# Alexander-H-Liu/End-to-end-ASR-Pytorch

Measured on AMD Instinct MI355X. Metric: audio frames/sec training (LAS+CTC, LibriSpeech 80-mel), higher is better.
Workload: dtype f32; 1 GPU; cfg3: {"B": 32, "T": 1600, "D": 80, "V": 5000, "L": 64}; global_batch=32, parallelism=dp1

## Files before the change

end-to-end-asr-pytorch_amd/csrc/core.cpp:

```cpp
#include "common.h"
#include "knobs.h"
#include <cstdlib>
#include <mutex>
#include <vector>

namespace {
struct DevInfo {
    int cu_count = 0;
    int lds_per_cu = 0;
    bool ok = false;
};
DevInfo g_dev[64];

struct ProfRec {
    hipEvent_t a, b;
    int id;
};
bool g_prof_on = false;
std::vector<ProfRec> g_pending;
double g_total_ms[PROF_NUM];
int64_t g_launches[PROF_NUM];
std::mutex g_mu;
hipEvent_t g_cur[PROF_NUM];
}

namespace {
AsrkKnobs g_knobs;
std::once_flag g_knobs_once;
int env_int(const char *name) {
    const char *e = getenv(name);
    return e ? atoi(e) : AsrkKnobs::UNSET;
}
int env_present(const char *name) { return getenv(name) ? 1 : AsrkKnobs::UNSET; }
void read_knobs() {
    AsrkKnobs &k = g_knobs;
    k.gemm_noskinny = env_present("ASRK_GEMM_NOSKINNY");
    k.skinny_sk = env_int("ASRK_SKINNY_SK");
    k.gemm_dbg = env_int("ASRK_GEMM_DBG");
    k.gemm_nofast = env_present("ASRK_GEMM_NOFAST");
    k.split_w256 = env_int("ASRK_SPLIT_W256");
    k.split_tail = env_int("ASRK_SPLIT_TAIL");
    k.fwd_mt = env_int("ASRK_FWD_MT");
    k.fwd_nt = env_int("ASRK_FWD_NT");
    k.rec_bf_mt4 = env_int("ASRK_REC_BF_MT4");
    k.bwd_ub = env_int("ASRK_BWD_UB");
    k.bwd_nt = env_int("ASRK_BWD_NT");
    k.fwd_poll = env_int("ASRK_FWD_POLL");
    k.fwd_presleep = env_int("ASRK_FWD_PRESLEEP");
    k.bwd_poll = env_int("ASRK_BWD_POLL");
    k.bwd_presleep = env_int("ASRK_BWD_PRESLEEP");
    k.dbg_noload = env_present("ASRK_DBG_NOLOAD");
    k.deterministic = env_int("ASRK_DETERMINISTIC");
}
}

const AsrkKnobs &asrk_knobs_() {
    std::call_once(g_knobs_once, read_knobs);
    return g_knobs;
}

extern "C" int asrk_version(void) { return 200; }

extern "C" const char *asrk_strerror(int rc) {
    switch (rc) {
        case ASRK_OK: return "ok";
        case ASRK_EINVAL: return "asrk: invalid argument";
        case ASRK_ESHAPE: return "asrk: shape not supported by the persistent gfx950 kernels";
        case ASRK_EWORKSPACE: return "asrk: workspace too small";
        case ASRK_EDEVICE: return "asrk: device lacks the CUs/LDS the persistent kernel needs";
        case ASRK_ETIMEOUT: return "asrk: in-kernel grid synchronisation timed out";
        default: break;
    }
    if (rc > 0) return hipGetErrorString((hipError_t)rc);
    return "asrk: unknown error";
}

extern "C" int asrk_init(int device) {
    if (device < 0 || device >= 64) return ASRK_EINVAL;
    (void)asrk_knobs_();
    if (!g_dev[device].ok) {
        hipDeviceProp_t prop;
        hipError_t e = hipGetDeviceProperties(&prop, device);
        if (e != hipSuccess) return (int)e > 0 ? -(1000 + (int)e) : ASRK_EDEVICE;
        g_dev[device].cu_count = prop.multiProcessorCount;
        g_dev[device].lds_per_cu = (int)prop.maxSharedMemoryPerMultiProcessor;
        g_dev[device].ok = true;
    }
    return g_dev[device].cu_count;
}

extern "C" int asrk_cu_count_(void) {
    int dev = 0;
    if (hipGetDevice(&dev) != hipSuccess) return 0;
    if (dev < 0 || dev >= 64) return 0;
    if (!g_dev[dev].ok) {
        if (asrk_init(dev) <= 0) return 0;
    }
    return g_dev[dev].cu_count;
}

static double g_work[PROF_NUM] = {0};

static unsigned g_prof_mask = 0xffffffffu;
extern "C" void asrk_profile_enable(int on) { g_prof_on = on != 0; }
extern "C" void asrk_profile_families(unsigned mask) { g_prof_mask = mask; }
static inline bool prof_live(int id) { return g_prof_on && id >= 0 && id < PROF_NUM && ((g_prof_mask >> id) & 1u); }

extern "C" void asrk_profile_reset(void) {
    std::lock_guard<std::mutex> lk(g_mu);
    for (auto &r : g_pending) {
        hipEventDestroy(r.a);
        hipEventDestroy(r.b);
    }
    g_pending.clear();
    for (int i = 0; i < PROF_NUM; ++i) {
        g_total_ms[i] = 0.0;
        g_launches[i] = 0;
        g_work[i] = 0.0;
    }
}

extern "C" void asrk_prof_work_(int id, double flops) {
    if (prof_live(id)) g_work[id] += flops;
}
extern "C" int asrk_profile_get_work(int id, double *flops) {
    if (id < 0 || id >= PROF_NUM || !flops) return ASRK_EINVAL;
    *flops = g_work[id];
    return ASRK_OK;
}

extern "C" void asrk_prof_begin_(int id, hipStream_t s) {
    if (!prof_live(id)) return;
    hipEvent_t a;
    if (hipEventCreate(&a) != hipSuccess) return;
    hipEventRecord(a, s);
    g_cur[id] = a;
}

extern "C" void asrk_prof_end_(int id, hipStream_t s) {
    if (!prof_live(id)) return;
    hipEvent_t b;
    if (hipEventCreate(&b) != hipSuccess) return;
    hipEventRecord(b, s);
    std::lock_guard<std::mutex> lk(g_mu);
    g_pending.push_back({g_cur[id], b, id});
}

extern "C" void asrk_prof_launches_(int id, int64_t n) {
    if (!prof_live(id)) return;
    std::lock_guard<std::mutex> lk(g_mu);
    g_launches[id] += n;
}

extern "C" int asrk_profile_get(int id, double *total_ms, int64_t *launches) {
    if (id < 0 || id >= PROF_NUM) return ASRK_EINVAL;
    std::lock_guard<std::mutex> lk(g_mu);
    for (auto &r : g_pending) {
        hipEventSynchronize(r.b);
        float ms = 0.f;
        if (hipEventElapsedTime(&ms, r.a, r.b) == hipSuccess) {
            g_total_ms[r.id] += ms;
            g_launches[r.id] += 1;
        }
        hipEventDestroy(r.a);
        hipEventDestroy(r.b);
    }
    g_pending.clear();
    if (total_ms) *total_ms = g_total_ms[id];
    if (launches) *launches = g_launches[id];
    return ASRK_OK;
}
```

end-to-end-asr-pytorch_amd/csrc/gemm_split.hip:

```cpp
#include "common.h"
#include "knobs.h"
#include <algorithm>
#include <climits>

extern "C" int asrk_cu_count_(void);

namespace {

typedef __bf16 bf16x8 __attribute__((ext_vector_type(8)));

constexpr int PIECE = 1024;

struct SplitGemmArgs {
    const unsigned char *Ap, *Bp;
    float *C;
    const float *bias, *bias2;
    int M, N, ldc;
    int KC;
    size_t rb_stride_a, rb_stride_b;
    int nk;
    int tiles_m, tiles_n;
    float alpha, beta;
    int slices, ldw;
    float *ws;
};

__device__ __forceinline__ void split8(const float (&v)[8], u32x4 (&w)[3]) {
    unsigned h[3][8];
#pragma unroll
    for (int e = 0; e < 8; ++e) {
        const float a = v[e];
        const __bf16 b0 = (__bf16)a;
        const float r1 = a - (float)b0;
        const __bf16 b1 = (__bf16)r1;
        const float r2 = r1 - (float)b1;
        const __bf16 b2 = (__bf16)r2;
        h[0][e] = __builtin_bit_cast(unsigned short, b0);
        h[1][e] = __builtin_bit_cast(unsigned short, b1);
        h[2][e] = __builtin_bit_cast(unsigned short, b2);
    }
#pragma unroll
    for (int p = 0; p < 3; ++p)
#pragma unroll
        for (int q = 0; q < 4; ++q) w[p][q] = h[p][2 * q] | (h[p][2 * q + 1] << 16);
}

template <bool VEC>
__global__ __launch_bounds__(256) void split_panel_kernel(const float *__restrict__ src, int ld, int R, int K,
                                                          unsigned char *__restrict__ dst, int KC, int RB,
                                                          size_t rb_stride) {
    constexpr int CHUNK = 3 * PIECE;
    const int lane = threadIdx.x & 63;
    const int KG = KC >> 2;
    const int64_t item = (int64_t)blockIdx.x * 4 + (threadIdx.x >> 6);
    if (item >= (int64_t)RB * KG) return;
    const int rb = (int)(item / KG), c0 = (int)(item - (int64_t)rb * KG) * 4;
    unsigned char *drb = dst + (size_t)rb * rb_stride;
    const int c = c0 + (lane & 3), k0 = c * 8;
#pragma unroll
    for (int it = 0; it < 4; ++it) {
        const int rl = it * 16 + (lane >> 2), row = rb * 64 + rl;
        float v[8];
        const float *s = src + (size_t)row * ld + k0;
        if (VEC && row < R && k0 + 8 <= K) {
            const f32x4 lo = *reinterpret_cast<const f32x4 *>(s), hi = *reinterpret_cast<const f32x4 *>(s + 4);
            v[0] = lo[0]; v[1] = lo[1]; v[2] = lo[2]; v[3] = lo[3];
            v[4] = hi[0]; v[5] = hi[1]; v[6] = hi[2]; v[7] = hi[3];
        } else {
#pragma unroll
            for (int e = 0; e < 8; ++e) v[e] = (row < R && k0 + e < K) ? s[e] : 0.f;
        }
        u32x4 w[3];
        split8(v, w);
        unsigned char *d = drb + (size_t)c * CHUNK + rl * 16;
#pragma unroll
        for (int p = 0; p < 3; ++p) *reinterpret_cast<u32x4 *>(d + p * PIECE) = w[p];
    }
}

template <int NCG>
__global__ __launch_bounds__(256) void split_panel_t_kernel(const float *__restrict__ src, int ld, int R, int K,
                                                            unsigned char *__restrict__ dst, int KC, int RB,
                                                            size_t rb_stride) {
    constexpr int CHUNK = 3 * PIECE;
    const int lane = threadIdx.x & 63, wave = __builtin_amdgcn_readfirstlane(threadIdx.x >> 6);
    const int64_t item = (int64_t)blockIdx.x * 4 + wave;
    const int KGn = KC / NCG;
    if (item >= (int64_t)RB * KGn) return;
    const int g = (int)(item / RB), rb = (int)(item - (int64_t)g * RB);
    const int c0 = g * NCG, k0 = c0 * 8, row = rb * 64 + lane;
    float v[NCG][8];
    const float *s = src + (size_t)k0 * ld + row;
    if (k0 + 8 * NCG <= K && rb * 64 + 64 <= R) {
#pragma unroll
        for (int cc = 0; cc < NCG; ++cc)
#pragma unroll
            for (int e = 0; e < 8; ++e) v[cc][e] = s[(size_t)(cc * 8 + e) * ld];
    } else {
#pragma unroll
        for (int cc = 0; cc < NCG; ++cc)
#pragma unroll
            for (int e = 0; e < 8; ++e)
                v[cc][e] = (row < R && k0 + cc * 8 + e < K) ? s[(size_t)(cc * 8 + e) * ld] : 0.f;
    }
    unsigned char *d = dst + (size_t)rb * rb_stride + (size_t)c0 * CHUNK + lane * 16;
#pragma unroll
    for (int cc = 0; cc < NCG; ++cc) {
        u32x4 w[3];
        split8(v[cc], w);
#pragma unroll
        for (int p = 0; p < 3; ++p) *reinterpret_cast<u32x4 *>(d + (size_t)cc * CHUNK + p * PIECE) = w[p];
    }
}

template <int N>
__device__ __forceinline__ void glds16_run(const unsigned char *g, unsigned voff, unsigned char *l) {
    static_assert(N >= 1 && N <= 4, "immediate offset range");
    const auto *gp = (const __attribute__((address_space(1))) unsigned char *)g + voff;
    auto *lp = (__attribute__((address_space(3))) void *)l;
    __builtin_amdgcn_global_load_lds(gp, lp, 16, 0, 0);
    if constexpr (N > 1) __builtin_amdgcn_global_load_lds(gp, lp, 16, PIECE, 0);
    if constexpr (N > 2) __builtin_amdgcn_global_load_lds(gp, lp, 16, 2 * PIECE, 0);
    if constexpr (N > 3) __builtin_amdgcn_global_load_lds(gp, lp, 16, 3 * PIECE, 0);
}

template <int N>
__device__ __forceinline__ void wait_vm() {
    static_assert(N >= 0 && N < 64, "vmcnt is a 6-bit field");
    __builtin_amdgcn_s_waitcnt((N & 15) | 0x70 | 0xF00 | (((N >> 4) & 3) << 14));
}
__device__ __forceinline__ void wait_lgkm0() { __builtin_amdgcn_s_waitcnt(0xC07F); }

template <int NC, int NST, bool SPEC, int WM, bool SK = false>
__global__ __launch_bounds__(SPEC ? (WM == 2 ? 512 : 704) : 256) void gemm_bf16x6_kernel(SplitGemmArgs p) {
    extern __shared__ __attribute__((aligned(1024))) unsigned char lds[];
    static_assert(WM == 2 || (WM == 4 && SPEC), "256-row tiles only with DMA waves");
    static_assert(!SK || NST >= 2, "the split-K epilogue transposes through a stage the last k-tile does not use");
    constexpr int NPL = 3, CHUNK = NPL * PIECE;
    constexpr int NCW = 2 * WM;
    constexpr int NRG = WM + 2;
    constexpr int RPD = WM == 2 ? 1 : 2;
    constexpr int REGION = NC * CHUNK;
    constexpr int STAGE = NRG * REGION;
    constexpr int LPT = NC * NPL * RPD;
    const int tid = threadIdx.x, lane = tid & 63;
    const int wave = __builtin_amdgcn_readfirstlane(tid >> 6);
    const int ntiles = p.tiles_m * p.tiles_n;
    const int slice = SK ? blockIdx.x / ntiles : 0, bid = SK ? blockIdx.x - slice * ntiles : blockIdx.x;
    const int kt0 = SK ? (int)((long)slice * p.nk / p.slices) : 0;
    const int nk = SK ? (int)((long)(slice + 1) * p.nk / p.slices) - kt0 : p.nk;
    const int q8 = ntiles >> 3, r8 = ntiles & 7, xcd = bid & 7, loc = bid >> 3;
    const int tile = (xcd < r8 ? xcd * (q8 + 1) : r8 * (q8 + 1) + (xcd - r8) * q8) + loc;
    constexpr int BAND = 8;
    const int band = tile / (BAND * p.tiles_m);
    const int band_w = min(BAND, p.tiles_n - band * BAND);
    const int in_band = tile - band * BAND * p.tiles_m;
    const int tm = in_band / band_w, tn = band * BAND + in_band % band_w;

    const bool loader = !SPEC || wave >= NCW, worker = !SPEC || wave < NCW;
    const int wr = worker ? wave >> 1 : 0, wc = wave & 1;
    const int ltm = tm, ltn = tn;
    const int r0 = (SPEC ? wave - NCW : wave) * RPD;
    const unsigned char *gsrc[RPD];
#pragma unroll
    for (int q = 0; q < RPD; ++q) {
        const int r = r0 + q;
        gsrc[q] = (r < WM ? p.Ap + (size_t)(ltm * WM + r) * p.rb_stride_a
                          : p.Bp + (size_t)(ltn * 2 + r - WM) * p.rb_stride_b);
        if (SK) gsrc[q] += (size_t)kt0 * REGION;
    }
    const unsigned voff = lane * 16;
    unsigned char *ldst = lds + r0 * REGION;
    static_assert((NC * NPL) % 4 == 0, "a region is issued as runs of four pieces");
    auto issue = [&](int kt, int stage) {
        unsigned char *l = ldst + stage * STAGE;
#pragma unroll
        for (int q = 0; q < RPD; ++q) {
            const unsigned char *g = gsrc[q] + (size_t)kt * REGION;
#pragma unroll
            for (int j = 0; j < NC * NPL; j += 4) glds16_run<4>(g + j * PIECE, voff, l + q * REGION + j * PIECE);
        }
    };

    f32x16 acc[2][2];
#pragma unroll
    for (int i = 0; i < 2; ++i)
#pragma unroll
        for (int j = 0; j < 2; ++j)
#pragma unroll
            for (int r = 0; r < 16; ++r) acc[i][j][r] = 0.f;

    const int frag_off = ((lane >> 5) * NPL) * PIECE + (lane & 31) * 16;
    const unsigned char *abase = lds + wr * REGION + frag_off;
    const unsigned char *bbase = lds + (WM + wc) * REGION + frag_off;
    constexpr int S = NC / 2;

    bf16x8 fa[2][2][NPL], fb[2][2][NPL];
    auto load_frags = [&](int buf, int stage, int ks) {
        const unsigned char *a_st = abase + stage * STAGE + ks * 2 * NPL * PIECE;
        const unsigned char *b_st = bbase + stage * STAGE + ks * 2 * NPL * PIECE;
#pragma unroll
        for (int i = 0; i < 2; ++i)
#pragma unroll
            for (int pl = 0; pl < NPL; ++pl) {
                fa[buf][i][pl] = *reinterpret_cast<const bf16x8 *>(a_st + pl * PIECE + i * 512);
                fb[buf][i][pl] = *reinterpret_cast<const bf16x8 *>(b_st + pl * PIECE + i * 512);
            }
        __builtin_amdgcn_sched_barrier(0);
    };
    auto step = [&](int buf, bool load, int lstage, int lks) {
        constexpr int NT = 6;
        constexpr int PA[6] = {2, 1, 0, 1, 0, 0};
        constexpr int PB[6] = {0, 1, 2, 0, 1, 0};
        constexpr int RPL[6] = {2, 0, 1, 1, 0, 2};
        const unsigned char *a_st = abase + lstage * STAGE + lks * 2 * NPL * PIECE;
        const unsigned char *b_st = bbase + lstage * STAGE + lks * 2 * NPL * PIECE;
        const int nb = buf ^ 1;
#pragma unroll
        for (int m = 0; m < 4 * NT; ++m) {
            const int t = m >> 2, i = (m >> 1) & 1, j = m & 1;
            acc[i][j] = __builtin_amdgcn_mfma_f32_32x32x16_bf16(fa[buf][i][PA[t]], fb[buf][j][PB[t]], acc[i][j], 0, 0, 0);
            __builtin_amdgcn_sched_barrier(0);
            if (load && m < 4 * NPL) {
                const int g = m >> 1, h = m & 1, pl = RPL[g];
                if ((g & 1) == 0) fa[nb][h][pl] = *reinterpret_cast<const bf16x8 *>(a_st + pl * PIECE + h * 512);
                else fb[nb][h][pl] = *reinterpret_cast<const bf16x8 *>(b_st + pl * PIECE + h * 512);
                __builtin_amdgcn_sched_barrier(0);
            }
        }
    };

    if (loader) {
#pragma unroll
        for (int s = 0; s < NST; ++s)
            if (s < nk) issue(s, s);
        const int later = min(NST - 1, nk - 1);
        if (NST > 3 && later >= 3) wait_vm<(NST > 3 ? 3 * LPT : 0)>();
        else if (NST > 2 && later == 2) wait_vm<(NST > 2 ? 2 * LPT : 0)>();
        else if (later == 1) wait_vm<LPT>();
        else wait_vm<0>();
    }
    __builtin_amdgcn_s_barrier();
    if (SPEC && !worker) {
        int stage = 0;
        for (int kt = 0; kt + 1 < nk; ++kt) {
            const int later = min(NST - 2, nk - 2 - kt);
            if (NST > 3 && later >= 2) wait_vm<(NST > 3 ? 2 * LPT : 0)>();
            else if (NST > 2 && later == 1) wait_vm<(NST > 2 ? LPT : 0)>();
            else wait_vm<0>();
            __builtin_amdgcn_s_barrier();
            if (kt + NST < nk) issue(kt + NST, stage);
            if (++stage == NST) stage = 0;
        }
        return;
    }
    load_frags(0, 0, 0);

    int stage = 0;
    static_assert(S >= 2 && S % 2 == 0, "fragment double buffer assumes an even number of steps per tile");
    for (int kt = 0; kt + 1 < nk; ++kt) {
#pragma unroll
        for (int ks = 0; ks < S - 1; ++ks) {
            wait_lgkm0();
            step(ks & 1, true, stage, ks + 1);
        }
        int nstage = stage + 1;
        if (nstage == NST) nstage = 0;
        const int later = min(NST - 2, nk - 2 - kt);
        wait_lgkm0();
        if (!SPEC) {
            if (NST > 3 && later >= 2) wait_vm<(NST > 3 ? 2 * LPT : 0)>();
            else if (NST > 2 && later == 1) wait_vm<(NST > 2 ? LPT : 0)>();
            else wait_vm<0>();
        }
        __builtin_amdgcn_s_barrier();
        if (!SPEC && kt + NST < nk) issue(kt + NST, stage);
        step((S - 1) & 1, true, nstage, 0);
        stage = nstage;
    }
    {
#pragma unroll
        for (int ks = 0; ks < S - 1; ++ks) {
            wait_lgkm0();
            step(ks & 1, true, stage, ks + 1);
        }
        wait_lgkm0();
        step((S - 1) & 1, false, 0, 0);
    }

    if constexpr (SK) {
        constexpr int PITCH = 36;
        static_assert(NCW * 32 * PITCH * 4 <= STAGE, "transposition images fit one stage");
        int fstage = stage + 1;
        if (fstage == NST) fstage = 0;
        float *img = reinterpret_cast<float *>(lds + fstage * STAGE) + wave * 32 * PITCH;
        float *wsl = p.ws + (size_t)slice * p.M * p.ldw;
        const int wrow0 = tm * 64 * WM + wr * 64, wcol0 = tn * 128 + wc * 64;
#pragma unroll
        for (int i = 0; i < 2; ++i)
#pragma unroll
            for (int j = 0; j < 2; ++j) {
#pragma unroll
                for (int r = 0; r < 16; ++r)
                    img[((r & 3) + 8 * (r >> 2) + 4 * (lane >> 5)) * PITCH + (lane & 31)] = acc[i][j][r];
                __builtin_amdgcn_fence(__ATOMIC_RELEASE, "wavefront");
                __builtin_amdgcn_wave_barrier();
                __builtin_amdgcn_fence(__ATOMIC_ACQUIRE, "wavefront");
#pragma unroll
                for (int q = 0; q < 4; ++q) {
                    const int idx = q * 64 + lane, rl = idx >> 3, c4 = (idx & 7) * 4;
                    const f32x4 v = *reinterpret_cast<const f32x4 *>(img + rl * PITCH + c4);
                    const int row = wrow0 + i * 32 + rl, col = wcol0 + j * 32 + c4;
                    if (row < p.M && col < p.ldw) *reinterpret_cast<f32x4 *>(wsl + (size_t)row * p.ldw + col) = v;
                }
                __builtin_amdgcn_fence(__ATOMIC_RELEASE, "wavefront");
                __builtin_amdgcn_wave_barrier();
                __builtin_amdgcn_fence(__ATOMIC_ACQUIRE, "wavefront");
            }
        return;
    }
    const int row0 = tm * 64 * WM + wr * 64 + 4 * (lane >> 5), col0 = tn * 128 + wc * 64 + (lane & 31);
#pragma unroll
    for (int j = 0; j < 2; ++j) {
        const int col = col0 + j * 32;
        if (col >= p.N) continue;
        float bsum = 0.f;
        if (p.bias) bsum += p.bias[col];
        if (p.bias2) bsum += p.bias2[col];
#pragma unroll
        for (int i = 0; i < 2; ++i)
#pragma unroll
            for (int r = 0; r < 16; ++r) {
                const int row = row0 + i * 32 + (r & 3) + 8 * (r >> 2);
                if (row >= p.M) continue;
                float *c = p.C + (size_t)row * p.ldc + col;
                float v = p.alpha * acc[i][j][r] + bsum;
                if (p.beta != 0.f) v += p.beta * *c;
                *c = v;
            }
    }
}

__global__ __launch_bounds__(256) void splitk_reduce_kernel(const float *__restrict__ ws, int slices, int M, int N,
                                                            int ldw, float alpha, float beta, float *__restrict__ C,
                                                            int ldc, const float *__restrict__ bias,
                                                            const float *__restrict__ bias2) {
    const int n4 = ldw >> 2;
    const int64_t idx = (int64_t)blockIdx.x * 256 + threadIdx.x;
    if (idx >= (int64_t)M * n4) return;
    const int row = (int)(idx / n4), col = (int)(idx - (int64_t)row * n4) * 4;
    const size_t plane = (size_t)M * ldw;
    const float *w = ws + (size_t)row * ldw + col;
    f32x4 a = *reinterpret_cast<const f32x4 *>(w);
    for (int s = 1; s < slices; ++s) a += *reinterpret_cast<const f32x4 *>(w + (size_t)s * plane);
#pragma unroll
    for (int e = 0; e < 4; ++e) {
        if (col + e >= N) break;
        float bsum = 0.f;
        if (bias) bsum += bias[col + e];
        if (bias2) bsum += bias2[col + e];
        float *c = C + (size_t)row * ldc + col + e;
        float v = alpha * a[e] + bsum;
        if (beta != 0.f) v += beta * *c;
        *c = v;
    }
}

template <int NST, int NDW>
__global__ __launch_bounds__((4 + NDW) * 64) void gemm_bf16x6_w256_kernel(SplitGemmArgs p, int rb_b, int BAND) {
    extern __shared__ __attribute__((aligned(1024))) unsigned char lds[];
    constexpr int NPL = 3, NC = 2, CHUNK = NPL * PIECE;
    constexpr int REGION = NC * CHUNK;
    constexpr int NRG = 6;
    constexpr int STAGE = NRG * REGION;
    constexpr int LPT = NRG * NC * NPL / NDW;
    static_assert(LPT * NDW == NRG * NC * NPL && (NDW == 3 || NDW == 4), "36 pieces per stage over 3 or 4 DMA waves");
    const int tid = threadIdx.x, lane = tid & 63;
    const int wave = __builtin_amdgcn_readfirstlane(tid >> 6);
    const int ntiles = p.tiles_m * p.tiles_n, bid = blockIdx.x;
    const int q8 = ntiles >> 3, r8 = ntiles & 7, xcd = bid & 7, loc = bid >> 3;
    const int tile = (xcd < r8 ? xcd * (q8 + 1) : r8 * (q8 + 1) + (xcd - r8) * q8) + loc;
    const int band = tile / (BAND * p.tiles_m);
    const int band_w = min(BAND, p.tiles_n - band * BAND);
    const int in_band = tile - band * BAND * p.tiles_m;
    const int tm = in_band / band_w, tn = band * BAND + in_band % band_w;
    const int nk = p.nk;

    if (wave >= 4) {
        const int d = wave - 4, first = d * LPT;
        constexpr int NRUN = LPT / 3;
        static_assert(NRUN * 3 == LPT, "runs of three pieces");
        const unsigned char *run_g[NRUN];
#pragma unroll
        for (int k = 0; k < NRUN; ++k) {
            const int idx = first + 3 * k, r = idx / (NC * NPL), j = idx - r * (NC * NPL);
            run_g[k] = (r < 2 ? p.Ap + (size_t)(tm * 2 + r) * p.rb_stride_a
                              : p.Bp + (size_t)min(tn * 4 + r - 2, rb_b - 1) * p.rb_stride_b) + j * PIECE;
        }
        const unsigned voff = lane * 16;
        unsigned char *ldst = lds + first * PIECE;
        auto issue = [&](int kt, int stage) {
            unsigned char *l = ldst + stage * STAGE;
            const size_t gk = (size_t)kt * REGION;
#pragma unroll
            for (int k = 0; k < NRUN; ++k) glds16_run<3>(run_g[k] + gk, voff, l + 3 * k * PIECE);
        };
#pragma unroll
        for (int s = 0; s < NST; ++s)
            if (s < nk) issue(s, s);
        {
            const int later = min(NST - 2, nk - 2);
            if (later >= 2) wait_vm<2 * LPT>();
            else if (later == 1) wait_vm<LPT>();
            else wait_vm<0>();
        }
        __builtin_amdgcn_s_barrier();
        int stage = 0;
        for (int kt = 0; kt < nk; ++kt) {
            const int later = min(NST - 2, nk - 2 - kt);
            if (later >= 2) wait_vm<2 * LPT>();
            else if (later == 1) wait_vm<LPT>();
            else wait_vm<0>();
            __builtin_amdgcn_s_barrier();
            if (kt + NST < nk) issue(kt + NST, stage);
            if (++stage == NST) stage = 0;
        }
        return;
    }

    const int wr = wave >> 1, wc = wave & 1;
    f32x16 acc[2][4];
#pragma unroll
    for (int i = 0; i < 2; ++i)
#pragma unroll
        for (int j = 0; j < 4; ++j)
#pragma unroll
            for (int r = 0; r < 16; ++r) acc[i][j][r] = 0.f;
    const int frag_off = ((lane >> 5) * NPL) * PIECE + (lane & 31) * 16;
    const unsigned char *abase = lds + wr * REGION + frag_off;
    const unsigned char *bbase = lds + (2 + wc * 2) * REGION + frag_off;
    bf16x8 fa1[2], fa2[2], fb1[4], fb2[4], fa0[2][2], fb0[2][4];
    auto rd_a1 = [&](bf16x8 &dst, int stage, int pl, int i) {
        dst = *reinterpret_cast<const bf16x8 *>(abase + stage * STAGE + pl * PIECE + i * 512);
    };
    auto rd_b1 = [&](bf16x8 &dst, int stage, int pl, int j) {
        dst = *reinterpret_cast<const bf16x8 *>(bbase + stage * STAGE + (j >> 1) * REGION + pl * PIECE + (j & 1) * 512);
    };
    auto rd_a = [&](bf16x8 (&dst)[2], int stage, int pl) {
#pragma unroll
        for (int i = 0; i < 2; ++i) rd_a1(dst[i], stage, pl, i);
    };
    auto rd_b = [&](bf16x8 (&dst)[4], int stage, int pl) {
#pragma unroll
        for (int j = 0; j < 4; ++j) rd_b1(dst[j], stage, pl, j);
    };
#define ASRK_TERM8(FA, FB)                                                                                 \
    do {                                                                                                   \
        _Pragma("unroll") for (int i = 0; i < 2; ++i) _Pragma("unroll") for (int j = 0; j < 4; ++j)         \
            acc[i][j] = __builtin_amdgcn_mfma_f32_32x32x16_bf16(FA[i], FB[j], acc[i][j], 0, 0, 0);          \
        __builtin_amdgcn_sched_barrier(0);                                                                 \
    } while (0)
#define ASRK_TERM8_RD(FA, FB, RD)                                                                          \
    do {                                                                                                   \
        _Pragma("unroll") for (int m = 0; m < 8; ++m) {                                                    \
            acc[m >> 2][m & 3] =                                                                           \
                __builtin_amdgcn_mfma_f32_32x32x16_bf16(FA[m >> 2], FB[m & 3], acc[m >> 2][m & 3], 0, 0, 0); \
            __builtin_amdgcn_sched_barrier(0);                                                             \
            RD(m);                                                                                         \
            __builtin_amdgcn_sched_barrier(0);                                                             \
        }                                                                                                  \
    } while (0)
#define ASRK_STEP(P)                                                                                       \
    do {                                                                                                   \
        int nstage = stage + 1;                                                                            \
        if (nstage == NST) nstage = 0;                                                                     \
        ASRK_TERM8(fa2, fb0[P]);                                                                           \
        wait_lgkm0();                                                                                      \
        __builtin_amdgcn_s_barrier();                                           \
        auto rd2 = [&](int m) {                                                                            \
            if (m == 0) rd_a1(fa2[0], nstage, 2, 0);                                                       \
            else if (m == 2) rd_a1(fa2[1], nstage, 2, 1);                                                  \
            else if (m == 4) rd_b1(fb0[1 - (P)][0], nstage, 0, 0);                                         \
            else if (m == 6) rd_b1(fb0[1 - (P)][1], nstage, 0, 1);                                         \
        };                                                                                                 \
        ASRK_TERM8_RD(fa0[P], fb2, rd2);                                                                   \
        auto rd3 = [&](int m) {                                                                            \
            if ((m & 1) == 0) rd_b1(fb2[m >> 1], nstage, 2, m >> 1);                                       \
        };                                                                                                 \
        ASRK_TERM8_RD(fa0[P], fb1, rd3);                                                                   \
        auto rd4 = [&](int m) {                                                                            \
            if (m == 0) rd_b1(fb0[1 - (P)][2], nstage, 0, 2);                                              \
            else if (m == 2) rd_b1(fb0[1 - (P)][3], nstage, 0, 3);                                         \
            else if (m == 4) rd_a1(fa0[1 - (P)][0], nstage, 0, 0);                                         \
            else if (m == 6) rd_a1(fa0[1 - (P)][1], nstage, 0, 1);                                         \
        };                                                                                                 \
        ASRK_TERM8_RD(fa1, fb1, rd4);                                                                      \
        auto rd5 = [&](int m) {                                                                            \
            if ((m & 1) == 0) rd_b1(fb1[m >> 1], nstage, 1, m >> 1);                                       \
        };                                                                                                 \
        ASRK_TERM8_RD(fa1, fb0[P], rd5);                                                                   \
        auto rd6 = [&](int m) {                                                                            \
            if (m == 1) rd_a1(fa1[0], nstage, 1, 0);                                                       \
            else if (m == 4) rd_a1(fa1[1], nstage, 1, 1);                                                  \
        };                                                                                                 \
        ASRK_TERM8_RD(fa0[P], fb0[P], rd6);                                                                \
        stage = nstage;                                                                                    \
    } while (0)

    __builtin_amdgcn_s_barrier();
    rd_a(fa2, 0, 2); rd_b(fb0[0], 0, 0); rd_a(fa0[0], 0, 0); rd_b(fb2, 0, 2); rd_b(fb1, 0, 1); rd_a(fa1, 0, 1);
    int stage = 0;
    for (int kt = 0; kt < nk; kt += 2) {
        ASRK_STEP(0);
        ASRK_STEP(1);
    }
#undef ASRK_STEP
#undef ASRK_TERM8_RD
#undef ASRK_TERM8

    const int row0 = tm * 128 + wr * 64 + 4 * (lane >> 5), col0 = tn * 256 + wc * 128 + (lane & 31);
#pragma unroll
    for (int j = 0; j < 4; ++j) {
        const int col = col0 + j * 32;
        if (col >= p.N) continue;
        float bsum = 0.f;
        if (p.bias) bsum += p.bias[col];
        if (p.bias2) bsum += p.bias2[col];
#pragma unroll
        for (int i = 0; i < 2; ++i)
#pragma unroll
            for (int r = 0; r < 16; ++r) {
                const int row = row0 + i * 32 + (r & 3) + 8 * (r >> 2);
                if (row >= p.M) continue;
                float *c = p.C + (size_t)row * p.ldc + col;
                float v = p.alpha * acc[i][j][r] + bsum;
                if (p.beta != 0.f) v += p.beta * *c;
                *c = v;
            }
    }
}

template <int NST, int NDW>
int launch_split_gemm_w256(const SplitGemmArgs &a, int rb_b, hipStream_t s) {
    constexpr int lds = NST * 6 * 2 * 3 * PIECE;
    auto kern = gemm_bf16x6_w256_kernel<NST, NDW>;
    static AsrkLdsLatch latch;
    ASRK_HIP(asrk_max_lds_once(latch, reinterpret_cast<const void *>(kern), lds));
    const int band = 2;
    hipLaunchKernelGGL(kern, dim3(a.tiles_m * a.tiles_n), dim3((4 + NDW) * 64), lds, s, a, rb_b, band);
    ASRK_LAUNCH_CHECK();
    return ASRK_OK;
}

template <int NC, int NST, bool SPEC, int WM, bool SK = false>
int launch_split_gemm(const SplitGemmArgs &a, hipStream_t s) {
    constexpr int lds = NST * (WM + 2) * NC * 3 * PIECE;
    auto kern = gemm_bf16x6_kernel<NC, NST, SPEC, WM, SK>;
    static AsrkLdsLatch latch;
    ASRK_HIP(asrk_max_lds_once(latch, reinterpret_cast<const void *>(kern), lds));
    hipLaunchKernelGGL(kern, dim3(a.tiles_m * a.tiles_n * (SK ? a.slices : 1)), dim3(SPEC ? (WM == 2 ? 512 : 704) : 256),
                       lds, s, a);
    ASRK_LAUNCH_CHECK();
    if (SK) {
        const int64_t items = (int64_t)a.M * (a.ldw >> 2);
        hipLaunchKernelGGL(splitk_reduce_kernel, dim3((unsigned)asrk_div_up64(items, 256)), dim3(256), 0, s, a.ws,
                           a.slices, a.M, a.N, a.ldw, a.alpha, a.beta, a.C, a.ldc, a.bias, a.bias2);
        ASRK_LAUNCH_CHECK();
    }
    return ASRK_OK;
}

}

namespace {
constexpr int SPLIT_NC = 4;
constexpr int NPL = 3;

struct PanelGeom {
    int KC, rb;
    size_t rb_stride, bytes;
};
PanelGeom panel_geom(int rows, int K, bool slack = false) {
    PanelGeom g;
    g.KC = (asrk_div_up(K, 8 * SPLIT_NC) + (slack ? 1 : 0)) * SPLIT_NC;
    g.rb = asrk_div_up(rows, 128) * 2;
    g.rb_stride = (size_t)g.KC * NPL * PIECE + 4352;
    g.bytes = (size_t)g.rb * g.rb_stride;
    return g;
}

int run_split(const float *src, int ld, int rows, int K, bool trans, unsigned char *dstp, const PanelGeom &g,
              hipStream_t s) {
    const dim3 grid((unsigned)asrk_div_up64((int64_t)g.rb * (g.KC / 4), 4));
    asrk_prof_work_(PROF_SPLIT, 4.0 * (double)rows * (double)K + 6.0 * (double)g.rb * 64.0 * (double)g.KC * 8.0);
    asrk_prof_begin_(PROF_SPLIT, s);
    if (trans) {
        hipLaunchKernelGGL((split_panel_t_kernel<4>), grid, dim3(256), 0, s, src, ld, rows, K, dstp, g.KC, g.rb, g.rb_stride);
    } else {
        const bool vec = (reinterpret_cast<uintptr_t>(src) & 15) == 0 && ld % 4 == 0;
        if (vec) hipLaunchKernelGGL((split_panel_kernel<true>), grid, dim3(256), 0, s, src, ld, rows, K, dstp, g.KC, g.rb, g.rb_stride);
        else hipLaunchKernelGGL((split_panel_kernel<false>), grid, dim3(256), 0, s, src, ld, rows, K, dstp, g.KC, g.rb, g.rb_stride);
    }
    asrk_prof_end_(PROF_SPLIT, s);
    ASRK_LAUNCH_CHECK();
    return ASRK_OK;
}

int auto_slices(int M, int N, int nk) {
    if (N >= 512) return 1;
    const int ncu = asrk_cu_count_() > 0 ? asrk_cu_count_() : 256;
    const long tiles = (long)asrk_div_up(M, 128) * asrk_div_up(N, 128);
    const long want = (ncu + tiles - 1) / tiles;
    return (int)std::max(1L, std::min(want, (long)(nk / 64)));
}

int run_panel_gemm(int M, int N, int nk, float alpha, const unsigned char *Ap, size_t stride_a,
                   const unsigned char *Bp, size_t stride_b, float beta, float *C, int ldc, const float *bias,
                   const float *bias2, hipStream_t s, int slices = 1, float *ws = nullptr) {
    const AsrkKnobs &kn = asrk_knobs_();
    SplitGemmArgs a;
    a.Ap = Ap; a.Bp = Bp; a.C = C; a.bias = bias; a.bias2 = bias2;
    a.M = M; a.N = N; a.ldc = ldc; a.KC = 0; a.nk = nk; a.rb_stride_a = stride_a; a.rb_stride_b = stride_b;
    a.tiles_m = asrk_div_up(M, 128); a.tiles_n = asrk_div_up(N, 128);
    a.alpha = alpha; a.beta = beta;
    a.slices = std::min(slices, nk); a.ldw = (N + 3) & ~3; a.ws = ws;
    if (a.slices > 1) return launch_split_gemm<4, 3, true, 2, true>(a, s);
    const int w256 = kn.get(kn.split_w256, 1);
    if (w256 && N >= 512) {
        const int tm = asrk_div_up(M, 128), tn = asrk_div_up(N, 256);
        const int ncu = asrk_cu_count_() > 0 ? asrk_cu_count_() : 256;
        if (w256 == 2 || (long)tm * tn >= 2L * ncu) {
            SplitGemmArgs b = a;
            b.tiles_m = tm; b.tiles_n = tn; b.nk = 2 * nk;
            const long tiles = (long)tm * tn, rem = tiles % ncu;
            const int tm1 = (int)((tiles - rem) / tn);
            if (w256 == 1 && rem > 0 && rem * 10 < 6L * ncu && tm1 > 0 && tm1 < tm && kn.get(kn.split_tail, 1)) {
                b.tiles_m = tm1; b.M = tm1 * 128;
                int rc = launch_split_gemm_w256<4, 4>(b, 2 * asrk_div_up(N, 128), s);
                if (rc != ASRK_OK) return rc;
                SplitGemmArgs c = a;
                c.Ap = a.Ap + (size_t)tm1 * 2 * a.rb_stride_a;
                c.C = a.C + (size_t)tm1 * 128 * ldc;
                c.M = M - tm1 * 128;
                c.tiles_m = asrk_div_up(c.M, 128);
                return launch_split_gemm<4, 3, true, 2>(c, s);
            }
            return launch_split_gemm_w256<4, 4>(b, 2 * asrk_div_up(N, 128), s);
        }
    }
    return launch_split_gemm<4, 3, true, 2>(a, s);
}
}

extern "C" size_t asrk_split_panel_stride_(int rows, int K) { return panel_geom(rows, K, true).rb_stride; }

extern "C" int asrk_gemm_takes_split(int M, int N, int K, int flags) {
    const int mode = flags & 3;
    if (mode == ASRK_GEMM_SPLIT_OFF || mode == 3 || K < 8 || M < 1 || N < 1) return 0;
    if (mode == ASRK_GEMM_SPLIT_AUTO) {
        const double hm = 2.0 * (double)M * (double)N / ((double)M + (double)N);
        const bool shallow_ok = K >= 64 && (double)M * (double)N >= 134217728.0;
        if (hm < 1500.0 || (K < 256 && !shallow_ok) || M < 256 || N < 256) return 0;
    }
    return 1;
}

extern "C" size_t asrk_gemm_ws_bytes(int M, int N, int K, int flags) {
    if (!asrk_gemm_takes_split(M, N, K, flags)) return 0;
    return panel_geom(M, K).bytes + panel_geom(N, K).bytes;
}

extern "C" int asrk_gemm_split_run_(int transA, int transB, int M, int N, int K, float alpha, const float *A,
                                    int lda, const float *B, int ldb, float beta, float *C, int ldc,
                                    const float *bias, const float *bias2, void *wsp, int flags, hipStream_t s) {
    const PanelGeom ga = panel_geom(M, K), gb = panel_geom(N, K);
    unsigned char *ws = reinterpret_cast<unsigned char *>(wsp);
    unsigned char *Ap = ws, *Bp = ws + ga.bytes;
    int rc = run_split(A, lda, M, K, transA != 0, Ap, ga, s);
    if (rc != ASRK_OK) return rc;
    rc = run_split(B, ldb, N, K, transB == 0, Bp, gb, s);
    if (rc != ASRK_OK) return rc;
    return run_panel_gemm(M, N, ga.KC / SPLIT_NC, alpha, Ap, ga.rb_stride, Bp, gb.rb_stride, beta, C, ldc, bias,
                          bias2, s);
}

extern "C" size_t asrk_split_panel_bytes(int rows, int K, int flags) {
    if (rows <= 0 || K <= 0 || flags != 0) return 0;
    return panel_geom(rows, K, true).bytes;
}

extern "C" int asrk_split_panel_f32(const float *src, int ld, int rows, int K, int trans, void *panel, int flags,
                                    void *stream) {
    if (!src || !panel || rows <= 0 || K <= 0 || ld < (trans ? rows : K) || flags != 0) return ASRK_EINVAL;
    if ((reinterpret_cast<uintptr_t>(panel) & 15) != 0) return ASRK_EINVAL;
    asrk_prof_begin_(PROF_GEMM, (hipStream_t)stream);
    const int rc = run_split(src, ld, rows, K, trans != 0, reinterpret_cast<unsigned char *>(panel),
                             panel_geom(rows, K, true), (hipStream_t)stream);
    asrk_prof_end_(PROF_GEMM, (hipStream_t)stream);
    return rc;
}

namespace {
struct PanelRange {
    const unsigned char *Ap, *Bp;
    size_t stride_a, stride_b;
    int nk;
};
int panel_range(int M, int N, int K, const void *A_panel, int a_rows, int a_K, int a_row0, int a_k0,
                const void *B_panel, int b_rows, int b_K, int b_row0, int b_k0, const float *C, int ldc, int flags,
                PanelRange &r) {
    if (M <= 0 || N <= 0 || K <= 0 || !A_panel || !B_panel || !C || ldc < N || flags != 0) return ASRK_EINVAL;
    if (a_row0 < 0 || b_row0 < 0 || a_k0 < 0 || b_k0 < 0 || a_row0 % 128 || b_row0 % 128 || a_k0 % 8 || b_k0 % 8)
        return ASRK_EINVAL;
    if (a_row0 + M > a_rows || b_row0 + N > b_rows || a_k0 + K > a_K || b_k0 + K > b_K) return ASRK_EINVAL;
    if (K % 32 != 0 && a_k0 + K != a_K && b_k0 + K != b_K) return ASRK_ESHAPE;
    const PanelGeom ga = panel_geom(a_rows, a_K, true), gb = panel_geom(b_rows, b_K, true);
    r.nk = asrk_div_up(K, 32);
    if (a_k0 / 8 + r.nk * SPLIT_NC > ga.KC || b_k0 / 8 + r.nk * SPLIT_NC > gb.KC) return ASRK_ESHAPE;
    const unsigned char *A0 = reinterpret_cast<const unsigned char *>(A_panel);
    const unsigned char *B0 = reinterpret_cast<const unsigned char *>(B_panel);
    r.Ap = A0 + (size_t)(a_row0 / 64) * ga.rb_stride + (size_t)(a_k0 / 8) * NPL * PIECE;
    r.Bp = B0 + (size_t)(b_row0 / 64) * gb.rb_stride + (size_t)(b_k0 / 8) * NPL * PIECE;
    r.stride_a = ga.rb_stride; r.stride_b = gb.rb_stride;
    return ASRK_OK;
}
}

extern "C" int asrk_gemm_panels_f32(int M, int N, int K, float alpha, const void *A_panel, int a_rows, int a_K,
                                    int a_row0, int a_k0, const void *B_panel, int b_rows, int b_K, int b_row0,
                                    int b_k0, float beta, float *C, int ldc, const float *bias,
                                    const float *bias2, int flags, void *stream) {
    PanelRange r;
    const int rc0 = panel_range(M, N, K, A_panel, a_rows, a_K, a_row0, a_k0, B_panel, b_rows, b_K, b_row0, b_k0, C, ldc,
                                flags, r);
    if (rc0 != ASRK_OK) return rc0;
    hipStream_t s = (hipStream_t)stream;
    asrk_prof_work_(PROF_GEMM, 2.0 * (double)M * (double)N * (double)K);
    asrk_prof_begin_(PROF_GEMM, s);
    const int rc = run_panel_gemm(M, N, r.nk, alpha, r.Ap, r.stride_a, r.Bp, r.stride_b, beta, C, ldc, bias, bias2, s);
    asrk_prof_end_(PROF_GEMM, s);
    return rc;
}

extern "C" size_t asrk_gemm_panels_splitk_ws_bytes(int M, int N, int splitk) {
    if (M <= 0 || N <= 0 || splitk < 0) return 0;
    const int n = splitk > 0 ? splitk : auto_slices(M, N, INT_MAX);
    return (size_t)n * (size_t)M * (size_t)((N + 3) & ~3) * sizeof(float);
}

extern "C" int asrk_gemm_panels_splitk_f32(int M, int N, int K, float alpha, const void *A_panel, int a_rows, int a_K,
                                           int a_row0, int a_k0, const void *B_panel, int b_rows, int b_K,
                                           int b_row0, int b_k0, float beta, float *C, int ldc, const float *bias,
                                           const float *bias2, int splitk, void *ws, size_t ws_bytes, int flags,
                                           void *stream) {
    if (splitk < 0 || !ws || (reinterpret_cast<uintptr_t>(ws) & 15) != 0) return ASRK_EINVAL;
    PanelRange r;
    const int rc0 = panel_range(M, N, K, A_panel, a_rows, a_K, a_row0, a_k0, B_panel, b_rows, b_K, b_row0, b_k0, C, ldc,
                                flags, r);
    if (rc0 != ASRK_OK) return rc0;
    const int slices = splitk > 0 ? splitk : auto_slices(M, N, r.nk);
    if (ws_bytes < asrk_gemm_panels_splitk_ws_bytes(M, N, slices)) return ASRK_EWORKSPACE;
    hipStream_t s = (hipStream_t)stream;
    asrk_prof_work_(PROF_GEMM, 2.0 * (double)M * (double)N * (double)K);
    asrk_prof_begin_(PROF_GEMM, s);
    const int rc = run_panel_gemm(M, N, r.nk, alpha, r.Ap, r.stride_a, r.Bp, r.stride_b, beta, C, ldc, bias, bias2, s,
                                  slices, reinterpret_cast<float *>(ws));
    asrk_prof_end_(PROF_GEMM, s);
    return rc;
}
```

end-to-end-asr-pytorch_amd/csrc/knobs.h:

```cpp
#pragma once

struct AsrkKnobs {
    static constexpr int UNSET = -0x7fffffff;
    int gemm_noskinny;
    int skinny_sk;
    int gemm_dbg;
    int gemm_nofast;
    int split_w256;
    int split_tail;
    int fwd_mt, fwd_nt;
    int rec_bf_mt4;
    int bwd_ub, bwd_nt;
    int fwd_poll, fwd_presleep;
    int bwd_poll, bwd_presleep;
    int dbg_noload;
    int deterministic;

    int get(int v, int dflt) const { return v == UNSET ? dflt : v; }
    bool is_set(int v) const { return v != UNSET; }
};

const AsrkKnobs &asrk_knobs_();
```

Before: 535,800 frames/s.

## Add 16x16x32 MFMA variants of split bf16x6 GEMM kernels for deep K

Adds new 128x128 and 128x256 split-bf16 GEMM kernels built on the 16x16x32 bf16 MFMA instruction. They interleave each MFMA with LDS fragment reads under scheduling barriers and split the waves into dedicated loader and worker groups. These kernels are selected by default when the K-panel count is at least 48, and can be overridden with an env knob. The aim is higher MFMA throughput and better overlap of LDS reads with math, at the cost of more register pressure and a large new code path.

Result: faster. 548,300 frames/s, median of 6 (+2.3%).

```diff
diff --git a/end-to-end-asr-pytorch_amd/csrc/core.cpp b/end-to-end-asr-pytorch_amd/csrc/core.cpp
--- a/end-to-end-asr-pytorch_amd/csrc/core.cpp
+++ b/end-to-end-asr-pytorch_amd/csrc/core.cpp
@@ -40,6 +40,7 @@
     k.gemm_nofast = env_present("ASRK_GEMM_NOFAST");
     k.split_w256 = env_int("ASRK_SPLIT_W256");
     k.split_tail = env_int("ASRK_SPLIT_TAIL");
+    k.split_mfma = env_int("ASRK_SPLIT_MFMA");
     k.fwd_mt = env_int("ASRK_FWD_MT");
     k.fwd_nt = env_int("ASRK_FWD_NT");
     k.rec_bf_mt4 = env_int("ASRK_REC_BF_MT4");
diff --git a/end-to-end-asr-pytorch_amd/csrc/gemm_split.hip b/end-to-end-asr-pytorch_amd/csrc/gemm_split.hip
--- a/end-to-end-asr-pytorch_amd/csrc/gemm_split.hip
+++ b/end-to-end-asr-pytorch_amd/csrc/gemm_split.hip
@@ -552,6 +552,345 @@
     return ASRK_OK;
 }
 
+#define ASRK_P16(FA, FB, ACC, RD)                                                                          \
+    do {                                                                                                   \
+        _Pragma("unroll") for (int m = 0; m < 16; ++m) {                                                   \
+            ACC[m >> 2][m & 3] =                                                                           \
+                __builtin_amdgcn_mfma_f32_16x16x32_bf16(FA[m >> 2], FB[m & 3], ACC[m >> 2][m & 3], 0, 0, 0); \
+            __builtin_amdgcn_sched_barrier(0);                                                             \
+            RD(m);                                                                                         \
+            __builtin_amdgcn_sched_barrier(0);                                                             \
+        }                                                                                                  \
+    } while (0)
+
+template <int START, int STRIDE>
+__device__ __forceinline__ void rd16_at(int m, bf16x8 (&slot)[4], const unsigned char *src) {
+    static_assert(START + 3 * STRIDE < 16, "inside one product");
+    const int i = (m - START) / STRIDE;
+    if (m >= START && i < 4 && START + i * STRIDE == m) slot[i] = *reinterpret_cast<const bf16x8 *>(src + i * 256);
+}
+__device__ __forceinline__ void rd16_all(bf16x8 (&slot)[4], const unsigned char *src) {
+#pragma unroll
+    for (int i = 0; i < 4; ++i) slot[i] = *reinterpret_cast<const bf16x8 *>(src + i * 256);
+}
+
+template <int P> struct StepSet { static constexpr int value = P; };
+
+template <bool SK>
+__global__ __launch_bounds__(512) void gemm_bf16x6_m16_kernel(SplitGemmArgs p) {
+    extern __shared__ __attribute__((aligned(1024))) unsigned char lds[];
+    constexpr int NPL = 3, NC = 4, NST = 3, CHUNK = NPL * PIECE;
+    constexpr int REGION = NC * CHUNK, STAGE = 4 * REGION, LPT = NC * NPL;
+    const int tid = threadIdx.x, lane = tid & 63;
+    const int wave = __builtin_amdgcn_readfirstlane(tid >> 6);
+    const int ntiles = p.tiles_m * p.tiles_n;
+    const int slice = SK ? blockIdx.x / ntiles : 0, bid = SK ? blockIdx.x - slice * ntiles : blockIdx.x;
+    const int kt0 = SK ? (int)((long)slice * p.nk / p.slices) : 0;
+    const int nk = SK ? (int)((long)(slice + 1) * p.nk / p.slices) - kt0 : p.nk;
+    const int q8 = ntiles >> 3, r8 = ntiles & 7, xcd = bid & 7, loc = bid >> 3;
+    const int tile = (xcd < r8 ? xcd * (q8 + 1) : r8 * (q8 + 1) + (xcd - r8) * q8) + loc;
+    constexpr int BAND = 8;
+    const int band = tile / (BAND * p.tiles_m);
+    const int band_w = min(BAND, p.tiles_n - band * BAND);
+    const int in_band = tile - band * BAND * p.tiles_m;
+    const int tm = in_band / band_w, tn = band * BAND + in_band % band_w;
+
+    const bool worker = wave < 4;
+    const int wr = worker ? wave >> 1 : 0, wc = wave & 1;
+    const int r0 = worker ? 0 : wave - 4;
+    const unsigned char *gsrc = (r0 < 2 ? p.Ap + (size_t)(tm * 2 + r0) * p.rb_stride_a
+                                        : p.Bp + (size_t)(tn * 2 + r0 - 2) * p.rb_stride_b) + (size_t)kt0 * REGION;
+    const unsigned voff = lane * 16;
+    unsigned char *ldst = lds + r0 * REGION;
+    auto issue = [&](int kt, int stage) {
+        const unsigned char *g = gsrc + (size_t)kt * REGION;
+        unsigned char *l = ldst + stage * STAGE;
+#pragma unroll
+        for (int j = 0; j < LPT; j += 4) glds16_run<4>(g + j * PIECE, voff, l + j * PIECE);
+    };
+
+    f32x4 acc[4][4];
+#pragma unroll
+    for (int i = 0; i < 4; ++i)
+#pragma unroll
+        for (int j = 0; j < 4; ++j)
+#pragma unroll
+            for (int r = 0; r < 4; ++r) acc[i][j][r] = 0.f;
+    const int frag_off = ((lane >> 4) * NPL) * PIECE + (lane & 15) * 16;
+    const unsigned char *abase = lds + wr * REGION + frag_off;
+    const unsigned char *bbase = lds + (2 + wc) * REGION + frag_off;
+    bf16x8 fa0[2][4], fa1[4], fa2[4], fb0[4], fb1[4], fb2[4];
+
+    if (!worker) {
+#pragma unroll
+        for (int s = 0; s < NST; ++s)
+            if (s < nk) issue(s, s);
+        const int later = min(NST - 1, nk - 1);
+        if (later >= 2) wait_vm<2 * LPT>();
+        else if (later == 1) wait_vm<LPT>();
+        else wait_vm<0>();
+    }
+    __builtin_amdgcn_s_barrier();
+    if (worker) {
+        rd16_all(fa0[0], abase); rd16_all(fb2, bbase + 2 * PIECE);
+        rd16_all(fa1, abase + PIECE); rd16_all(fb1, bbase + PIECE); rd16_all(fa2, abase + 2 * PIECE);
+        __builtin_amdgcn_sched_barrier(0);
+    }
+
+    int stage = 0, kt = 0;
+    auto step = [&](auto set) {
+        constexpr int P = decltype(set)::value, Q = 1 - P;
+        int nstage = stage + 1;
+        if (nstage == NST) nstage = 0;
+        const unsigned char *bc = bbase + stage * STAGE;
+        const unsigned char *an = abase + nstage * STAGE, *bn = bbase + nstage * STAGE;
+        if (worker) {
+            auto rd1 = [&](int m) { rd16_at<0, 4>(m, fb0, bc); };
+            ASRK_P16(fa0[P], fb2, acc, rd1);
+            auto rd2 = [&](int) {};
+            ASRK_P16(fa1, fb1, acc, rd2);
+            wait_lgkm0();
+        } else {
+            if (nk - 2 - kt >= 1) wait_vm<LPT>();
+            else wait_vm<0>();
+        }
+        __builtin_amdgcn_s_barrier();
+        if (worker) {
+            auto rd3 = [&](int m) { rd16_at<0, 4>(m, fb2, bn + 2 * PIECE); };
+            ASRK_P16(fa0[P], fb1, acc, rd3);
+            auto rd4 = [&](int m) { rd16_at<0, 4>(m, fa0[Q], an); };
+            ASRK_P16(fa2, fb0, acc, rd4);
+            auto rd5 = [&](int m) { rd16_at<0, 4>(m, fa2, an + 2 * PIECE); rd16_at<2, 4>(m, fb1, bn + PIECE); };
+            ASRK_P16(fa1, fb0, acc, rd5);
+            auto rd6 = [&](int m) { rd16_at<0, 2>(m, fa1, an + PIECE); };
+            ASRK_P16(fa0[P], fb0, acc, rd6);
+        } else if (kt + NST < nk) {
+            issue(kt + NST, stage);
+        }
+        stage = nstage;
+        ++kt;
+    };
+    while (kt < nk) {
+        step(StepSet<0>());
+        if (kt < nk) step(StepSet<1>());
+    }
+    if (!worker) return;
+
+    if constexpr (SK) {
+        constexpr int PITCH = 68;
+        static_assert(4 * 16 * PITCH * 4 <= STAGE, "transposition images fit one stage");
+        float *img = reinterpret_cast<float *>(lds) + wave * 16 * PITCH;
+        float *wsl = p.ws + (size_t)slice * p.M * p.ldw;
+        const int wrow0 = tm * 128 + wr * 64, wcol0 = tn * 128 + wc * 64;
+        wait_lgkm0();
+#pragma unroll
+        for (int i = 0; i < 4; ++i) {
+#pragma unroll
+            for (int j = 0; j < 4; ++j)
+#pragma unroll
+                for (int r = 0; r < 4; ++r) img[(4 * (lane >> 4) + r) * PITCH + j * 16 + (lane & 15)] = acc[i][j][r];
+            __builtin_amdgcn_fence(__ATOMIC_RELEASE, "wavefront");
+            __builtin_amdgcn_wave_barrier();
+            __builtin_amdgcn_fence(__ATOMIC_ACQUIRE, "wavefront");
+#pragma unroll
+            for (int q = 0; q < 4; ++q) {
+                const int idx = q * 64 + lane, rl = idx >> 4, c4 = (idx & 15) * 4;
+                const f32x4 v = *reinterpret_cast<const f32x4 *>(img + rl * PITCH + c4);
+                const int row = wrow0 + i * 16 + rl, col = wcol0 + c4;
+                if (row < p.M && col < p.ldw) *reinterpret_cast<f32x4 *>(wsl + (size_t)row * p.ldw + col) = v;
+            }
+            __builtin_amdgcn_fence(__ATOMIC_RELEASE, "wavefront");
+            __builtin_amdgcn_wave_barrier();
+            __builtin_amdgcn_fence(__ATOMIC_ACQUIRE, "wavefront");
+        }
+        return;
+    }
+    const int row0 = tm * 128 + wr * 64 + 4 * (lane >> 4), col0 = tn * 128 + wc * 64 + (lane & 15);
+#pragma unroll
+    for (int j = 0; j < 4; ++j) {
+        const int col = col0 + j * 16;
+        if (col >= p.N) continue;
+        float bsum = 0.f;
+        if (p.bias) bsum += p.bias[col];
+        if (p.bias2) bsum += p.bias2[col];
+#pragma unroll
+        for (int i = 0; i < 4; ++i)
+#pragma unroll
+            for (int r = 0; r < 4; ++r) {
+                const int row = row0 + i * 16 + r;
+                if (row >= p.M) continue;
+                float *c = p.C + (size_t)row * p.ldc + col;
+                float v = p.alpha * acc[i][j][r] + bsum;
+                if (p.beta != 0.f) v += p.beta * *c;
+                *c = v;
+            }
+    }
+}
+
+template <int NDW>
+__global__ __launch_bounds__((4 + NDW) * 64) void gemm_bf16x6_w256_m16_kernel(SplitGemmArgs p, int rb_b, int BAND) {
+    extern __shared__ __attribute__((aligned(1024))) unsigned char lds[];
+    constexpr int NPL = 3, NC = 2, CHUNK = NPL * PIECE;
+    constexpr int REGION = NC * CHUNK, NRG = 6, STAGE = NRG * REGION, PAIR = 2 * STAGE;
+    constexpr int LPT = NRG * NC * NPL / NDW, NRUN = LPT / 3;
+    static_assert(LPT * NDW == NRG * NC * NPL && NRUN * 3 == LPT, "36 pieces per stage, runs of three");
+    const int tid = threadIdx.x, lane = tid & 63;
+    const int wave = __builtin_amdgcn_readfirstlane(tid >> 6);
+    const int ntiles = p.tiles_m * p.tiles_n, bid = blockIdx.x;
+    const int q8 = ntiles >> 3, r8 = ntiles & 7, xcd = bid & 7, loc = bid >> 3;
+    const int tile = (xcd < r8 ? xcd * (q8 + 1) : r8 * (q8 + 1) + (xcd - r8) * q8) + loc;
+    const int band = tile / (BAND * p.tiles_m);
+    const int band_w = min(BAND, p.tiles_n - band * BAND);
+    const int in_band = tile - band * BAND * p.tiles_m;
+    const int tm = in_band / band_w, tn = band * BAND + in_band % band_w;
+    const int ns = p.nk >> 1;
+
+    const bool worker = wave < 4;
+    const int first = (worker ? 0 : wave - 4) * LPT;
+    const unsigned char *run_g[NRUN];
+#pragma unroll
+    for (int k = 0; k < NRUN; ++k) {
+        const int idx = first + 3 * k, r = idx / (NC * NPL), j = idx - r * (NC * NPL);
+        run_g[k] = (r < 2 ? p.Ap + (size_t)(tm * 2 + r) * p.rb_stride_a
+                          : p.Bp + (size_t)min(tn * 4 + r - 2, rb_b - 1) * p.rb_stride_b) + j * PIECE;
+    }
+    const unsigned voff = lane * 16;
+    unsigned char *ldst = lds + first * PIECE;
+    auto issue_pair = [&](int s, int slot) {
+#pragma unroll
+        for (int h = 0; h < 2; ++h) {
+            unsigned char *l = ldst + slot * PAIR + h * STAGE;
+            const size_t gk = (size_t)(2 * s + h) * REGION;
+#pragma unroll
+            for (int k = 0; k < NRUN; ++k) glds16_run<3>(run_g[k] + gk, voff, l + 3 * k * PIECE);
+        }
+    };
+
+    const int wr = worker ? wave >> 1 : 0, wc = wave & 1;
+    f32x4 acc0[4][4], acc1[4][4];
+#pragma unroll
+    for (int i = 0; i < 4; ++i)
+#pragma unroll
+        for (int j = 0; j < 4; ++j)
+#pragma unroll
+            for (int r = 0; r < 4; ++r) acc0[i][j][r] = acc1[i][j][r] = 0.f;
+    const int frag_off = (lane >> 5) * STAGE + (((lane >> 4) & 1) * NPL) * PIECE + (lane & 15) * 16;
+    const unsigned char *abase = lds + wr * REGION + frag_off;
+    const unsigned char *bbase = lds + (2 + wc * 2) * REGION + frag_off;
+    bf16x8 fa0[2][4], fa1[4], fa2[4], fb0[4], fb1[4], fb2[4];
+
+    if (!worker) {
+        issue_pair(0, 0);
+        if (ns > 1) {
+            issue_pair(1, 1);
+            wait_vm<2 * LPT>();
+        } else {
+            wait_vm<0>();
+        }
+    }
+    __builtin_amdgcn_s_barrier();
+    if (worker) {
+        rd16_all(fa0[0], abase); rd16_all(fb2, bbase + 2 * PIECE);
+        rd16_all(fa1, abase + PIECE); rd16_all(fb1, bbase + PIECE); rd16_all(fa2, abase + 2 * PIECE);
+        __builtin_amdgcn_sched_barrier(0);
+    }
+
+    int s = 0;
+    auto step = [&](auto set) {
+        constexpr int P = decltype(set)::value, Q = 1 - P;
+        const unsigned char *bc = bbase + P * PAIR;
+        const unsigned char *an = abase + Q * PAIR, *bn = bbase + Q * PAIR;
+        auto rd0 = [&](int) {};
+        if (worker) {
+            auto rd1 = [&](int m) { rd16_at<0, 4>(m, fb0, bc); };
+            ASRK_P16(fa0[P], fb2, acc0, rd1);
+            auto rd2 = [&](int m) { rd16_at<0, 4>(m, fb2, bc + REGION + 2 * PIECE); };
+            ASRK_P16(fa1, fb1, acc0, rd2);
+            ASRK_P16(fa0[P], fb1, acc0, rd0);
+            auto rd4 = [&](int m) { rd16_at<0, 4>(m, fb1, bc + REGION + PIECE); };
+            ASRK_P16(fa2, fb0, acc0, rd4);
+            ASRK_P16(fa1, fb0, acc0, rd0);
+            ASRK_P16(fa0[P], fb0, acc0, rd0);
+            wait_lgkm0();
+            auto rd7 = [&](int m) { rd16_at<0, 4>(m, fb0, bc + REGION); };
+            ASRK_P16(fa0[P], fb2, acc1, rd7);
+            ASRK_P16(fa1, fb1, acc1, rd0);
+            wait_lgkm0();
+        } else {
+            wait_vm<0>();
+        }
+        __builtin_amdgcn_s_barrier();
+        if (worker) {
+            auto rd9 = [&](int m) { rd16_at<0, 4>(m, fb2, bn + 2 * PIECE); };
+            ASRK_P16(fa0[P], fb1, acc1, rd9);
+            auto rd10 = [&](int m) { rd16_at<0, 4>(m, fa0[Q], an); };
+            ASRK_P16(fa2, fb0, acc1, rd10);
+            auto rd11 = [&](int m) { rd16_at<0, 4>(m, fa2, an + 2 * PIECE); rd16_at<2, 4>(m, fb1, bn + PIECE); };
+            ASRK_P16(fa1, fb0, acc1, rd11);
+            auto rd12 = [&](int m) { rd16_at<0, 2>(m, fa1, an + PIECE); };
+            ASRK_P16(fa0[P], fb0, acc1, rd12);
+        } else if (s + 2 < ns) {
+            issue_pair(s + 2, P);
+        }
+        ++s;
+    };
+    while (s < ns) {
+        step(StepSet<0>());
+        if (s < ns) step(StepSet<1>());
+    }
+    if (!worker) return;
+
+    const int row0 = tm * 128 + wr * 64 + 4 * (lane >> 4), col0 = tn * 256 + wc * 128 + (lane & 15);
+#pragma unroll
+    for (int j = 0; j < 8; ++j) {
+        const int col = col0 + j * 16;
+        if (col >= p.N) continue;
+        float bsum = 0.f;
+        if (p.bias) bsum += p.bias[col];
+        if (p.bias2) bsum += p.bias2[col];
+#pragma unroll
+        for (int i = 0; i < 4; ++i)
+#pragma unroll
+            for (int r = 0; r < 4; ++r) {
+                const int row = row0 + i * 16 + r;
+                if (row >= p.M) continue;
+                float *c = p.C + (size_t)row * p.ldc + col;
+                float v = p.alpha * (j < 4 ? acc0[i][j & 3][r] : acc1[i][j & 3][r]) + bsum;
+                if (p.beta != 0.f) v += p.beta * *c;
+                *c = v;
+            }
+    }
+}
+#undef ASRK_P16
+
+template <bool SK>
+int launch_split_gemm_m16(const SplitGemmArgs &a, hipStream_t s) {
+    constexpr int lds = 3 * 4 * 4 * 3 * PIECE;
+    auto kern = gemm_bf16x6_m16_kernel<SK>;
+    static AsrkLdsLatch latch;
+    ASRK_HIP(asrk_max_lds_once(latch, reinterpret_cast<const void *>(kern), lds));
+    hipLaunchKernelGGL(kern, dim3(a.tiles_m * a.tiles_n * (SK ? a.slices : 1)), dim3(512), lds, s, a);
+    ASRK_LAUNCH_CHECK();
+    if (SK) {
+        const int64_t items = (int64_t)a.M * (a.ldw >> 2);
+        hipLaunchKernelGGL(splitk_reduce_kernel, dim3((unsigned)asrk_div_up64(items, 256)), dim3(256), 0, s, a.ws,
+                           a.slices, a.M, a.N, a.ldw, a.alpha, a.beta, a.C, a.ldc, a.bias, a.bias2);
+        ASRK_LAUNCH_CHECK();
+    }
+    return ASRK_OK;
+}
+
+int launch_split_gemm_w256_m16(const SplitGemmArgs &a, int rb_b, hipStream_t s) {
+    constexpr int lds = 4 * 6 * 2 * 3 * PIECE;
+    auto kern = gemm_bf16x6_w256_m16_kernel<4>;
+    static AsrkLdsLatch latch;
+    ASRK_HIP(asrk_max_lds_once(latch, reinterpret_cast<const void *>(kern), lds));
+    const int band = 2;
+    hipLaunchKernelGGL(kern, dim3(a.tiles_m * a.tiles_n), dim3(512), lds, s, a, rb_b, band);
+    ASRK_LAUNCH_CHECK();
+    return ASRK_OK;
+}
+
 template <int NC, int NST, bool SPEC, int WM, bool SK = false>
 int launch_split_gemm(const SplitGemmArgs &a, hipStream_t s) {
     constexpr int lds = NST * (WM + 2) * NC * 3 * PIECE;
@@ -575,6 +914,7 @@
 namespace {
 constexpr int SPLIT_NC = 4;
 constexpr int NPL = 3;
+constexpr int SPLIT_MFMA16_MIN_NK = 48;
 
 struct PanelGeom {
     int KC, rb;
@@ -624,7 +964,10 @@
     a.tiles_m = asrk_div_up(M, 128); a.tiles_n = asrk_div_up(N, 128);
     a.alpha = alpha; a.beta = beta;
     a.slices = std::min(slices, nk); a.ldw = (N + 3) & ~3; a.ws = ws;
-    if (a.slices > 1) return launch_split_gemm<4, 3, true, 2, true>(a, s);
+    const bool m16 = kn.is_set(kn.split_mfma) ? kn.split_mfma == 16 : nk >= SPLIT_MFMA16_MIN_NK;
+    const bool m16_sk = kn.is_set(kn.split_mfma) && kn.split_mfma == 16;
+    const bool m16_128 = m16, m16_w256 = m16;
+    if (a.slices > 1) return m16_sk ? launch_split_gemm_m16<true>(a, s) : launch_split_gemm<4, 3, true, 2, true>(a, s);
     const int w256 = kn.get(kn.split_w256, 1);
     if (w256 && N >= 512) {
         const int tm = asrk_div_up(M, 128), tn = asrk_div_up(N, 256);
@@ -636,19 +979,21 @@
             const int tm1 = (int)((tiles - rem) / tn);
             if (w256 == 1 && rem > 0 && rem * 10 < 6L * ncu && tm1 > 0 && tm1 < tm && kn.get(kn.split_tail, 1)) {
                 b.tiles_m = tm1; b.M = tm1 * 128;
-                int rc = launch_split_gemm_w256<4, 4>(b, 2 * asrk_div_up(N, 128), s);
+                int rc = m16_w256 ? launch_split_gemm_w256_m16(b, 2 * asrk_div_up(N, 128), s)
+                                  : launch_split_gemm_w256<4, 4>(b, 2 * asrk_div_up(N, 128), s);
                 if (rc != ASRK_OK) return rc;
                 SplitGemmArgs c = a;
                 c.Ap = a.Ap + (size_t)tm1 * 2 * a.rb_stride_a;
                 c.C = a.C + (size_t)tm1 * 128 * ldc;
                 c.M = M - tm1 * 128;
                 c.tiles_m = asrk_div_up(c.M, 128);
-                return launch_split_gemm<4, 3, true, 2>(c, s);
+                return m16_128 ? launch_split_gemm_m16<false>(c, s) : launch_split_gemm<4, 3, true, 2>(c, s);
             }
-            return launch_split_gemm_w256<4, 4>(b, 2 * asrk_div_up(N, 128), s);
-        }
-    }
-    return launch_split_gemm<4, 3, true, 2>(a, s);
+            return m16_w256 ? launch_split_gemm_w256_m16(b, 2 * asrk_div_up(N, 128), s)
+                            : launch_split_gemm_w256<4, 4>(b, 2 * asrk_div_up(N, 128), s);
+        }
+    }
+    return m16_128 ? launch_split_gemm_m16<false>(a, s) : launch_split_gemm<4, 3, true, 2>(a, s);
 }
 }
 
diff --git a/end-to-end-asr-pytorch_amd/csrc/knobs.h b/end-to-end-asr-pytorch_amd/csrc/knobs.h
--- a/end-to-end-asr-pytorch_amd/csrc/knobs.h
+++ b/end-to-end-asr-pytorch_amd/csrc/knobs.h
@@ -8,6 +8,7 @@
     int gemm_nofast;
     int split_w256;
     int split_tail;
+    int split_mfma;
     int fwd_mt, fwd_nt;
     int rec_bf_mt4;
     int bwd_ub, bwd_nt;
```
